# williamyang98/ViterbiDecoderCpp

Hardware: AMD Instinct MI355X
Metric: decoded Mbit/s (= ACS trellis steps/s), update()+chainback(), bit-exact vs scalar reference (higher is better)
Workload: dtype u16

## Files before the change

viterbidecodercpp_amd/csrc/kernels_reg.hpp:

```cpp
#pragma once
#include <hip/hip_runtime.h>
#include <stdint.h>

#include <type_traits>
#include <utility>

#include "common.hpp"

namespace vit {

typedef uint32_t u32;
typedef unsigned short u16x2_t __attribute__((ext_vector_type(2)));
typedef short s16x2_t __attribute__((ext_vector_type(2)));

#define VIT_DEV __device__ __forceinline__

VIT_DEV u32 pk_add(u32 a, u32 b) {
    return __builtin_bit_cast(u32, (u16x2_t)(__builtin_bit_cast(u16x2_t, a) + __builtin_bit_cast(u16x2_t, b)));
}
VIT_DEV u32 pk_sub(u32 a, u32 b) {
    return __builtin_bit_cast(u32, (u16x2_t)(__builtin_bit_cast(u16x2_t, a) - __builtin_bit_cast(u16x2_t, b)));
}
VIT_DEV u32 pk_max_s(u32 a, u32 b) {
    return __builtin_bit_cast(u32, __builtin_elementwise_max(__builtin_bit_cast(s16x2_t, a), __builtin_bit_cast(s16x2_t, b)));
// ... 869 lines not shown
                        constexpr int KV = SP::tail_kind(v % PER);
                        u32 fin;
                        if constexpr (KV == 1) fin = __builtin_amdgcn_perm(pend_acc, pend_f1, SELX32);
                        else if constexpr (KV == 2) fin = __builtin_amdgcn_perm(pend_acc, pend_f1, SELX16);
                        else if constexpr (KV == 3) fin = pend_f1;
                        else if constexpr (KV == 4) fin = __builtin_amdgcn_perm(pend_f1, pend_f2, SELX16);
                        else fin = __builtin_amdgcn_perm(pend_f1, pend_f2, SELX32);
                        dq[v % SPS] = fin;
                        if constexpr (v % SPS == SPS - 1)
                            ws_blk[(v / SPS) * 64 + lane] = make_uint4(dq[0], dq[1], dq[2], dq[3]);
                    };
                    constexpr int KU = SP::tail_kind(UP);
                    constexpr bool DEFER = !GUARDED;
                    if constexpr (DEFER && u > 0) {
                        if constexpr (SP::tail_kind((u - 1) % PER) != 0) finish_tail(std::integral_constant<int, u - 1>{});
                    }
                    if constexpr (KU == 0) {
                        dq[u % SPS] = acc[0];
                        if constexpr (u % SPS == SPS - 1)
                            ws_blk[(u / SPS) * 64 + lane] = make_uint4(dq[0], dq[1], dq[2], dq[3]);
                    } else {
                        pend_acc = acc[0];
                        if constexpr (KU == 1) pend_f1 = (u32)__builtin_amdgcn_ds_bpermute((int)XADDR32, (int)acc[0]);
                        else if constexpr (KU == 2) pend_f1 = (u32)__builtin_amdgcn_ds_bpermute((int)XADDR16, (int)acc[0]);
                        else pend_f1 = (u32)__builtin_amdgcn_ds_bpermute((int)LSWADDR, (int)acc[0]);
                        if constexpr (KU == 4) pend_f2 = (u32)__builtin_amdgcn_ds_bpermute((int)(LSWADDR ^ 128u), (int)acc[0]);
                        if constexpr (KU == 5) pend_f2 = (u32)__builtin_amdgcn_ds_bpermute((int)(LSWADDR ^ 64u), (int)acc[0]);
                        if constexpr (!DEFER) finish_tail(uc);
                    }
                }
                {
                    bool any;
                    if constexpr (EARLY_TEST) {
                        any = early_any != 0;
                    } else if constexpr (NREG >= 64) {
                        const u32 maskq0 = lane < 16 ? BIAS2 : 0u;
                        any = __builtin_amdgcn_ballot_w64(((pk_sub_sat_s_uniform(THRM1B2, m[0]) | FORCE) & maskq0) != 0) != 0;
                    } else {
                        any = __builtin_amdgcn_ballot_w64(pk_max_s(m[0], TLANE) != TCMP) != 0;
                    }
                    if constexpr (NREG >= 64) {
                    if (__builtin_expect(any, 0)) {
                        const u32 maskq = (SP::LANE_BITS == 0 || lane < 16) ? BIAS2 : 0u;
                        const u32 need2 = (pk_sub_sat_s_uniform(THRM1B2, m[0]) | FORCE) & maskq;
                        const u32 nq = SP::LANE_BITS ? (u32)__shfl((int)need2, (int)g) : need2;
                        const u32 msk = ((nq & 0x8000u) ? 0x0000FFFFu : 0u) | ((nq & 0x80000000u) ? 0xFFFF0000u : 0u);
                        u32 mn = m[0];
                        static_for<NREG - 1>([&](auto rc) __attribute__((always_inline)) {
                            mn = pk_min_s(mn, m[decltype(rc)::value + 1]);
                        });
                        if constexpr (SP::LANE_BITS) {
                            mn = pk_min_s(mn, (u32)__shfl_xor((int)mn, 16));
                            mn = pk_min_s(mn, (u32)__shfl_xor((int)mn, 32));
                        }
                        const u32 sub = (mn ^ BIAS2) & msk;
                        static_for<NREG>([&](auto rc) __attribute__((always_inline)) {
                            constexpr int r = decltype(rc)::value;
                            m[r] = pk_sub(m[r], sub);
                        });
                        rsA += (uint64_t)((sub & 0xFFFFu) >> SHIFT);
                        rsB += (uint64_t)((sub >> 16) >> SHIFT);
                    }
                    } else
                    if (__builtin_expect(any, 0)) {
                        u32 mn = m[0];
                        static_for<NREG - 1>([&](auto rc) __attribute__((always_inline)) {
                            mn = pk_min_s(mn, m[decltype(rc)::value + 1]);
                        });
                        u32 sub;
                        if constexpr (SP::LANE_BITS) {
                            const int16_t thr = (int16_t)(uint16_t)(THRM1B2 & 0xFFFFu);
                            uint64_t tA = __builtin_amdgcn_ballot_w64((int16_t)(uint16_t)(m[0] & 0xFFFFu) > thr);
                            uint64_t tB = __builtin_amdgcn_ballot_w64((int16_t)(uint16_t)(m[0] >> 16) > thr);
                            if (a.cfg.threshold == 0) tA = tB = 0xFFFFull;
                            tA &= 0xFFFFull; tB &= 0xFFFFull;
                            tA |= tA << 16; tA |= tA << 32;
                            tB |= tB << 16; tB |= tB << 32;
                            auto s16 = __builtin_amdgcn_permlane16_swap(mn, mn, false, false);
                            mn = pk_min_s(s16[0], s16[1]);
                            auto s32 = __builtin_amdgcn_permlane32_swap(mn, mn, false, false);
                            mn = pk_min_s(s32[0], s32[1]);
                            const u32 unb = mn ^ BIAS2;
                            u32 sa, sb;
                            asm("v_cndmask_b32_e64 %0, 0, %1, %2" : "=v"(sa) : "v"(unb), "s"(tA));
                            asm("v_cndmask_b32_e64 %0, 0, %1, %2" : "=v"(sb) : "v"(unb), "s"(tB));
                            sub = (sa & 0x0000FFFFu) | (sb & 0xFFFF0000u);
                        } else {
                            const u32 need2 = pk_sub_sat_s_uniform(THRM1B2, m[0]) | FORCE;
                            const u32 msk = ((need2 & 0x8000u) ? 0x0000FFFFu : 0u) | ((need2 & 0x80000000u) ? 0xFFFF0000u : 0u);
                            sub = (mn ^ BIAS2) & msk;
                        }
#ifndef VIT_REG_FOLD
#define VIT_REG_FOLD 1
#endif
                        constexpr bool FOLD = VIT_REG_FOLD && SP::LANE_BITS != 0 && !BMCHUNK && !SPLIT && 2 * NPF < NREG;
                        bool folded = false;
                        if constexpr (FOLD) {
                            if ((!GUARDED && u + 1 < U) || t0 + (u32)u + 1u < a.t_end) {
                                static_for<NPF>([&](auto pc) __attribute__((always_inline)) {
                                    constexpr int pp = decltype(pc)::value;
                                    E[(u + 1) & 1][pp] = pk_sub(E[(u + 1) & 1][pp], sub);
                                    EB[(u + 1) & 1][pp] = pk_sub(EB[(u + 1) & 1][pp], sub);
                                });
                                folded = true;
                            }
                        }
                        if (!folded) {
                            static_for<NREG>([&](auto rc) __attribute__((always_inline)) {
                                constexpr int r = decltype(rc)::value;
                                m[r] = pk_sub(m[r], sub);
                            });
                        }
                        rsA += (uint64_t)((sub & 0xFFFFu) >> SHIFT);
                        rsB += (uint64_t)((sub >> 16) >> SHIFT);
                    }
                }
                } else if constexpr (BMCHUNK) {
                    if constexpr (u % GROUP == GROUP - 1) {
                        constexpr int Jb = u / GROUP;
                        constexpr int sl = (Jb + 1) % NG;
                        bm_produce(std::integral_constant<int, GROUP * (Jb + 1)>{}, std::integral_constant<int, sl>{});
                        load_group(t0 + (u32)(GROUP * (Jb + 1 + NG)), std::integral_constant<int, sl>{});
                    }
                    if constexpr (GENERIC) {
                        gen_chunk_row(std::integral_constant<int, u + 1>{}, std::integral_constant<int, 0>{});
                        gen_chunk_row(std::integral_constant<int, u + 1>{}, std::integral_constant<int, 1>{});
                    }
                    static_for<AHEAD>([&](auto ac) __attribute__((always_inline)) { bm_fetch_chunk(std::integral_constant<int, u + 1>{}, ac); });
                }
            }
        });
    };
    if constexpr (RESUME) {
        for (; t0 < a.t_end; t0 += U, ws_blk += (U / SPS) * 64) {
            if (t0 >= T_BEGIN && t0 + U <= a.t_end) block(std::false_type{});
            else block(std::true_type{});
        }
    } else {
        __builtin_amdgcn_s_waitcnt(0x0F70);
        for (; t0 + U <= a.t_end; t0 += U, ws_blk += (U / SPS) * 64) block(std::false_type{});
        if (t0 < a.t_end) block(std::true_type{});
    }

    if constexpr (DW != 4) {
        if (a.t_end % SPS != 0) ws_tile[(size_t)(a.t_end / SPS) * 64 + lane] = make_uint4(dq[0], dq[1], dq[2], dq[3]);
    }

    if (a.metrics_out) {
        const int ph = (int)(a.t_end % SB);
        const int lu = (int)((a.t_end + (u32)PER - 1u) % (u32)PER);
        constexpr size_t N = (size_t)1 << SB;
        static_for<NREG>([&](auto rc) __attribute__((always_inline)) {
            constexpr u32 r = decltype(rc)::value;
            const u32 x = X3 ? SP::slot3(lu, q, r) : ((q << REG_BITS) | r);
            const u32 s = ((x << ph) | (x >> (SB - ph))) & SP::SMASK;
            const u32 v = m[r] ^ BIAS2;
            if (SHIFT) {
                if (validA) ((uint8_t*)a.metrics_out)[(size_t)fA * N + s] = (uint8_t)((v & 0xFFFFu) >> 8);
                if (validB) ((uint8_t*)a.metrics_out)[(size_t)fB * N + s] = (uint8_t)(v >> 24);
            } else {
                if (validA) ((uint16_t*)a.metrics_out)[(size_t)fA * N + s] = (uint16_t)(v & 0xFFFFu);
                if (validB) ((uint16_t*)a.metrics_out)[(size_t)fB * N + s] = (uint16_t)(v >> 16);
            }
        });
    }
    if (a.renorm_sum && q == 0) {
        if (validA) a.renorm_sum[fA] = rsA;
        if (validB) a.renorm_sum[fB] = rsB;
    }
}

struct RegChainbackArgs {
    const uint4* ws;
    size_t ws_tile_stride;
    uint8_t* out;
    const u32* end_state;
    u32 frames, L;
    u32 wave_priority;
};

template <class SP>
VIT_DEV void reg_chainback_coop_body(const RegChainbackArgs& a) {
    static_assert(SP::LANE_BITS == 2 && SP::DW * SP::SPS == 4 && SP::NREG >= 32, "K = 8, 9 layout");
    constexpr int SB = SP::SB, NREG = SP::NREG, REG_BITS = SP::REG_BITS, DW = SP::DW, SPS = SP::SPS;
    constexpr int IGN = SB < 8 ? SB : 8;
    constexpr int SHIFT_STATE = 8 - IGN, SHIFT_TAIL = SB - IGN, TOTAL_BITS = SB + SHIFT_STATE;
    constexpr int PASS = 16;
    constexpr int NBUF = PASS / SPS;
    constexpr int K0 = (((7 - SB) % 8) + 8) % 8;

    const int lane = threadIdx.x & 63;
    const u32 g = lane & 15, q = lane >> 4;
    const size_t tile = blockIdx.x;
    const u32 fA_raw = (u32)tile * 32 + g, fB_raw = fA_raw + 16;
    const bool validA = fA_raw < a.frames, validB = fB_raw < a.frames;
    const u32 fA = validA ? fA_raw : a.frames - 1, fB = validB ? fB_raw : a.frames - 1;
    const uint4* rows = a.ws + tile * a.ws_tile_stride + lane;
    const size_t out_stride = ((size_t)a.L + 7) / 8;
    uint8_t* outA = a.out + (size_t)fA * out_stride;
    uint8_t* outB = a.out + (size_t)fB * out_stride;

    u32 regA = (a.end_state ? (a.end_state[fA] & SP::SMASK) : 0u) << SHIFT_STATE;
    u32 regB = (a.end_state ? (a.end_state[fB] & SP::SMASK) : 0u) << SHIFT_STATE;

    auto trace = [&](u32& reg, const uint4& v, u32 half, u32 ph1, u32 sub) __attribute__((always_inline)) {
        const u32 state = reg >> SHIFT_STATE;
        const u32 x = ((state >> ph1) | (state << (SB - ph1))) & SP::SMASK;
        const u32 qs = x >> REG_BITS, rs = x & (NREG - 1);
        const u32 pos = 32u * (u32)DW * sub + rs + (rs & ~7u) + 8u * half;
        const uint64_t lo64 = ((uint64_t)v.y << 32) | v.x, hi64 = ((uint64_t)v.w << 32) | v.z;
        const uint64_t w64 = (pos & 64u) ? hi64 : lo64;
        const u32 mine = (u32)(w64 >> (pos & 63u)) & 1u;
        const u32 bit = (u32)__shfl((int)mine, (int)(qs * 16 + g));
        reg = (reg >> 1) | (bit << (TOTAL_BITS - 1));
    };
    auto emit = [&](u32 jb) __attribute__((always_inline)) {
        if (q == 0) {
            outA[jb] = (uint8_t)((regA >> SHIFT_TAIL) & 0xFFu);
            outB[jb] = (uint8_t)((regB >> SHIFT_TAIL) & 0xFFu);
        }
    };
    auto slow_step = [&](int t) __attribute__((always_inline)) {
        const uint4 v = rows[(size_t)(t / SPS) * 64];
        const u32 ph1 = (u32)((t + 1) % SB);
        trace(regA, v, 0u, ph1, (u32)(t % SPS));
        trace(regB, v, 1u, ph1, (u32)(t % SPS));
        const int j = t - SB;
        if ((j & 7) == 0) emit((u32)j >> 3);
    };

    int t = (int)a.L - 1 + SB;
    while (t >= SB && (t & 7) != 7) slow_step(t--);
    if (t >= SB && t - (PASS - 1) >= SB) {
        uint4 buf[NBUF];
#pragma unroll
        for (int b = 0; b < NBUF; ++b) buf[b] = rows[(size_t)(t / SPS - b) * 64];
        constexpr int BPP = PASS / 8;
        constexpr int KI = 128 / BPP;
        __shared__ u32 obufA[32 * 64], obufB[32 * 64];
        typedef u32 u32_unaligned __attribute__((aligned(1)));
        u32 ph_run = (u32)((t + 1) % SB);
        while (t - (PASS - 1) >= SB) {
            __builtin_amdgcn_s_waitcnt(0x0F70);
            int it = 0;
            for (; it < KI && t - (PASS - 1) >= SB; ++it, t -= PASS) {
#pragma unroll
                for (int b = 0; b < NBUF; ++b) {
#pragma unroll
                    for (int sidx = SPS - 1; sidx >= 0; --sidx) {
                        const int k = b * SPS + (SPS - 1 - sidx);
                        const u32 ph1 = SB == 8 ? (u32)((8 - (k % 8)) % 8) : ph_run;
                        trace(regA, buf[b], 0u, ph1, (u32)sidx);
                        trace(regB, buf[b], 1u, ph1, (u32)sidx);
                        if (SB != 8) ph_run = ph_run == 0 ? SB - 1 : ph_run - 1;
                        if (k % 8 == K0) {
                            const int slot = 127 - (it * BPP + k / 8);
                            ((uint8_t*)obufA)[(slot >> 2) * 256 + lane * 4 + (slot & 3)] = (uint8_t)((regA >> SHIFT_TAIL) & 0xFFu);
                            ((uint8_t*)obufB)[(slot >> 2) * 256 + lane * 4 + (slot & 3)] = (uint8_t)((regB >> SHIFT_TAIL) & 0xFFu);
                        }
                    }
                    asm volatile("" : "+v"(regA), "+v"(regB) : : "memory");
                    const int nxt = t / SPS - b - NBUF;
                    buf[b] = rows[(size_t)(nxt < 0 ? 0 : nxt) * 64];
                    __builtin_amdgcn_sched_barrier(0);
                }
            }
            if (q == 0) {
                const int nbytes = it * BPP;
                const u32 jb_lo = (u32)(t + PASS - (K0 + 8) - SB) >> 3;
                int sl = 128 - nbytes;
                for (; (sl & 3) != 0 && sl < 128; ++sl) {
                    outA[jb_lo + (u32)(sl - (128 - nbytes))] = ((const uint8_t*)obufA)[(sl >> 2) * 256 + lane * 4 + (sl & 3)];
                    outB[jb_lo + (u32)(sl - (128 - nbytes))] = ((const uint8_t*)obufB)[(sl >> 2) * 256 + lane * 4 + (sl & 3)];
                }
                for (; sl < 128; sl += 4) {
                    *(u32_unaligned*)(outA + jb_lo + (u32)(sl - (128 - nbytes))) = obufA[(sl >> 2) * 64 + lane];
                    *(u32_unaligned*)(outB + jb_lo + (u32)(sl - (128 - nbytes))) = obufB[(sl >> 2) * 64 + lane];
                }
            }
        }
    }
    while (t >= SB) slow_step(t--);
}

#ifndef VIT_REG_CB_RING_DEPTH_K7
#define VIT_REG_CB_RING_DEPTH_K7 4
#endif
constexpr int reg_cb_ring_depth(int nreg, int R) { return nreg == 16 ? (R >= 4 ? 2 : VIT_REG_CB_RING_DEPTH_K7) : 8; }
constexpr int reg_cb_ring_flush_iters(int nreg, int R) { return (nreg == 16 && R >= 4) ? 8 : 16; }
#ifndef VIT_REG_CB_STAGGER
#define VIT_REG_CB_STAGGER 0
#endif
constexpr unsigned reg_cb_ring_slot_bytes() { return 4096u + 4u * (unsigned)VIT_REG_CB_STAGGER; }
constexpr unsigned reg_cb_ring_lds_bytes(int nreg, int R) {
    return (unsigned)reg_cb_ring_depth(nreg, R) * reg_cb_ring_slot_bytes() + (unsigned)reg_cb_ring_flush_iters(nreg, R) * 512u;
}
template <class SP>
VIT_DEV void reg_chainback_ring_body(const RegChainbackArgs& a) {
    static_assert(SP::LANE_BITS == 2 && (SP::NREG == 16 || SP::NREG == 64) && SP::DW * SP::SPS == 4 && SP::SB <= 8, "K = 7, 9 layouts");
    constexpr int SB = SP::SB, REG_BITS = SP::REG_BITS, DW = SP::DW, SPS = SP::SPS;
    constexpr int IGN = SB < 8 ? SB : 8;
    constexpr int SHIFT_STATE = 8 - IGN;
    static_assert(SB - IGN == 0, "... and its low byte is the output byte (shift_tail = 0)");
    constexpr int ITER = 32;
    constexpr int ROWS_IT = ITER / SPS;
    constexpr int D = reg_cb_ring_depth(SP::NREG, SP::R);
    static_assert(ROWS_IT % D == 0, "ring slots are compile-time constants");
    constexpr int KI = reg_cb_ring_flush_iters(SP::NREG, SP::R);
    constexpr int CT = (ITER - 1 + SB) % ITER;
    static_assert(reg_cb_ring_lds_bytes(SP::NREG, SP::R) == D * reg_cb_ring_slot_bytes() + 2 * KI * 64 * 4, "launch size of the ring kernels");
    extern __shared__ uint4 reg_cb_dyn_lds[];
    uint4* const ring = reg_cb_dyn_lds;
    u32* const obuf = (u32*)((char*)reg_cb_dyn_lds + D * reg_cb_ring_slot_bytes());
    typedef __attribute__((address_space(3))) void lds_void_t;
    typedef __attribute__((address_space(1))) const void glb_void_t;
    typedef u32 u32_unaligned __attribute__((aligned(1)));

    const int lane = threadIdx.x & 63;
    const u32 n_tiles = (a.frames + 31u) >> 5;
    const u32 jt = (u32)lane >> 4, g = (u32)lane & 15u;
    const u32 tl_raw = blockIdx.x * 4u + jt;
    const u32 tl = tl_raw < n_tiles ? tl_raw : n_tiles - 1;
    const u32 fA = tl * 32u + g < a.frames ? tl * 32u + g : a.frames - 1;
    const u32 fB = tl * 32u + g + 16u < a.frames ? tl * 32u + g + 16u : a.frames - 1;
    const size_t out_stride = ((size_t)a.L + 7) / 8;
    uint8_t* outA = a.out + (size_t)fA * out_stride;
    uint8_t* outB = a.out + (size_t)fB * out_stride;
    const uint8_t* my_rows = (const uint8_t*)(a.ws + (size_t)tl * a.ws_tile_stride);
    const u32 src_off = (u32)lane * 16u;
    const u32 pair_base = jt * (1024u + (u32)VIT_REG_CB_STAGGER) + g * 16u;

    int t = (int)a.L - 1 + SB;
    const u32 esA = a.end_state ? (a.end_state[fA] & SP::SMASK) : 0u, esB = a.end_state ? (a.end_state[fB] & SP::SMASK) : 0u;
    u32 RA = esA << (24 + SHIFT_STATE), RB = esB << (24 + SHIFT_STATE);
    u32 ph = (u32)(t + 1) % (u32)SB;
    u32 xA = ((esA >> ph) | (esA << (SB - ph))) & SP::SMASK, xB = ((esB >> ph) | (esB << (SB - ph))) & SP::SMASK;
    u32 pos = (SB - ph) % SB;

    auto byte_of = [&](u32 x, u32 base) __attribute__((always_inline)) -> u32 {
        return base + 256u * __builtin_amdgcn_ubfe(x, REG_BITS, 2) + 2u * __builtin_amdgcn_ubfe(x, 3, REG_BITS - 3);
    };
    auto step_back = [&](u32& R, u32& x, u32 byte, u32 p) __attribute__((always_inline)) {
        const u32 bit = __builtin_amdgcn_ubfe(byte, x & 7u, 1);
        R = (R >> 1) | (bit << 31);
        x = (x & ~(1u << p)) | (bit << p);
    };
    auto slow_step = [&](int tt) __attribute__((always_inline)) {
        const uint8_t* row = my_rows + (size_t)(tt / SPS) * 1024u + (u32)(tt % SPS) * (4u * DW);
        const u32 bA = row[byte_of(xA, g * 16u)], bB = row[byte_of(xB, g * 16u) + 1u];
        step_back(RA, xA, bA, pos);
        step_back(RB, xB, bB, pos);
        pos = pos == SB - 1 ? 0u : pos + 1u;
        const int j = tt - SB;
        if ((j & 7) == 0) { outA[j >> 3] = (uint8_t)(RA >> 24); outB[j >> 3] = (uint8_t)(RB >> 24); }
    };

    while (t >= SB && (t & (ITER - 1)) != CT) slow_step(t--);
    if (t - (ITER - 1) >= SB) {
        const uint8_t* tb[4];
#pragma unroll
        for (int jj = 0; jj < 4; ++jj) {
            const u32 tr = blockIdx.x * 4u + (u32)jj;
            tb[jj] = (const uint8_t*)(a.ws + (size_t)(tr < n_tiles ? tr : n_tiles - 1) * a.ws_tile_stride);
        }
        typedef __attribute__((address_space(3))) uint8_t lds_u8_t;
        u32 ring_lds = (u32)(uintptr_t)(lds_u8_t*)ring;
        asm volatile("" : "+s"(ring_lds));
        auto fill = [&](int slot, int row) __attribute__((always_inline)) {
            const u32 vo = src_off + (u32)(row < 0 ? 0 : row) * 1024u;
#pragma unroll
            for (int jj = 0; jj < 4; ++jj)
                __builtin_amdgcn_global_load_lds((glb_void_t*)(tb[jj] + vo), (lds_void_t*)(lds_u8_t*)(uintptr_t)(ring_lds + (u32)slot * reg_cb_ring_slot_bytes() + (u32)jj * (1024u + (u32)VIT_REG_CB_STAGGER)), 16, 0, 0);
        };
        constexpr int S0 = (CT / SPS) % D;
#pragma unroll
        for (int k = 0; k < D; ++k) fill((S0 - k + D) % D, t / SPS - k);
        const uint8_t* ring_b = (const uint8_t*)ring;
        while (t - (ITER - 1) >= SB) {
            __builtin_amdgcn_s_waitcnt(0x0F70);
            const int t0 = t;
            int it = 0;
            for (; it < KI && t - (ITER - 1) >= SB; ++it, t -= ITER) {
#pragma unroll
                for (int pk = 0; pk < ITER; ++pk) {
                    const int cs = CT - pk;
                    const int rk = CT / SPS - (cs >= 0 ? cs / SPS : -((-cs + SPS - 1) / SPS));
                    const int sidx = ((cs % SPS) + SPS) % SPS;
                    const int slot = ((S0 - rk) % D + D) % D;
                    constexpr int NV = 4 * (D - 1);
                    __builtin_amdgcn_s_waitcnt(0x0F70 | (NV & 15) | ((NV >> 4) << 14));
                    const u32 wA = ring_b[slot * (int)reg_cb_ring_slot_bytes() + sidx * 4 * DW + byte_of(xA, pair_base)];
                    const u32 wB = ring_b[slot * (int)reg_cb_ring_slot_bytes() + sidx * 4 * DW + 1 + byte_of(xB, pair_base)];
                    if constexpr (ITER % SB == 0) {
                        const u32 p = (u32)((SB - (((CT - pk + 1) % SB) + SB) % SB) % SB);
                        step_back(RA, xA, wA, p);
                        step_back(RB, xB, wB, p);
                    } else {
                        step_back(RA, xA, wA, pos);
                        step_back(RB, xB, wB, pos);
                        pos = pos == SB - 1 ? 0u : pos + 1u;
                    }
                    if (sidx == 0) {
                        asm volatile("" : "+v"(RA), "+v"(RB), "+v"(xA), "+v"(xB) : : "memory");
                        fill(slot, (t - pk) / SPS - D);
                        __builtin_amdgcn_sched_barrier(0);
                    }
                }
                obuf[it * 64 + lane] = __builtin_amdgcn_perm(RA, RA, 0x00010203u);
                obuf[(KI + it) * 64 + lane] = __builtin_amdgcn_perm(RB, RB, 0x00010203u);
            }
            for (int i = 0; i < it; ++i) {
                const u32 jb = (u32)(t0 - ITER * i - (ITER - 1) - SB) >> 3;
                *(u32_unaligned*)(outA + jb) = obuf[i * 64 + lane];
                *(u32_unaligned*)(outB + jb) = obuf[(KI + i) * 64 + lane];
            }
        }
        __builtin_amdgcn_s_waitcnt(0x0F70);
        if constexpr (ITER % SB == 0) pos = (SB - (u32)(t + 1) % (u32)SB) % SB;
    }
    while (t >= SB) slow_step(t--);
}

template <class SP>
VIT_DEV void reg_chainback16_body(const RegChainbackArgs& a) {
    static_assert(SP::NREG == 16 && SP::DW == 1 && SP::SPS == 4 && SP::SB == 6, "K = 7 layout");
    constexpr int SB = SP::SB;
    constexpr int IGN = SB < 8 ? SB : 8;
    constexpr int SHIFT_STATE = 8 - IGN;
    static_assert(SB - IGN == 0, "shift_tail = 0: the output byte is the 8-bit register itself");
    constexpr int NBUF = 8;

    const int lane = threadIdx.x & 63;
    const u32 n_tiles = (a.frames + 31u) >> 5;
    const u32 p_raw = blockIdx.x * 64 + lane;
    const u32 tile = (p_raw >> 4) < n_tiles ? (p_raw >> 4) : n_tiles - 1, g = p_raw & 15u;
    const u32 fA = tile * 32u + g < a.frames ? tile * 32u + g : a.frames - 1;
    const u32 fB = tile * 32u + g + 16u < a.frames ? tile * 32u + g + 16u : a.frames - 1;
    const uint4* rows = a.ws + (size_t)tile * a.ws_tile_stride + g;
    const size_t out_stride = ((size_t)a.L + 7) / 8;
    uint8_t* outA = a.out + (size_t)fA * out_stride;
    uint8_t* outB = a.out + (size_t)fB * out_stride;
    constexpr u32 SELA = 0x06040200u, SELB = 0x07050301u;

    const u32 esA = a.end_state ? (a.end_state[fA] & SP::SMASK) : 0u, esB = a.end_state ? (a.end_state[fB] & SP::SMASK) : 0u;
    u32 regA = esA << (24 + SHIFT_STATE), regB = esB << (24 + SHIFT_STATE);
    const u32 ph_top = ((u32)a.L + (u32)SB) % (u32)SB;
    u32 xA = ((esA >> ph_top) | (esA << (SB - ph_top))) & SP::SMASK, xB = ((esB >> ph_top) | (esB << (SB - ph_top))) & SP::SMASK;

    auto chase1 = [&](u32& reg, u32& x, u32 lo, u32 hi, u32 p) __attribute__((always_inline)) {
        const u32 w = x > 31u ? hi : lo;
        const u32 bit = __builtin_amdgcn_ubfe(w, x, 1);
        reg = (reg >> 1) | (bit << 31);
        x = (x & ~(1u << p)) | (bit << p);
    };
    auto chase = [&](u32 d0, u32 d1, u32 d2, u32 d3, u32 p) __attribute__((always_inline)) {
        chase1(regA, xA, __builtin_amdgcn_perm(d1, d0, SELA), __builtin_amdgcn_perm(d3, d2, SELA), p);
        chase1(regB, xB, __builtin_amdgcn_perm(d1, d0, SELB), __builtin_amdgcn_perm(d3, d2, SELB), p);
    };
    auto pos_of = [](int t) __attribute__((always_inline)) -> u32 { return (u32)((SB - (t + 1) % SB) % SB); };
    auto emit = [&](u32 jb) __attribute__((always_inline)) {
        outA[jb] = (uint8_t)(regA >> 24);
        outB[jb] = (uint8_t)(regB >> 24);
    };
    auto slow_step = [&](int t) __attribute__((always_inline)) {
        const u32* r32 = (const u32*)(rows + (size_t)(t >> 2) * 64) + (t & 3);
        chase(r32[0], r32[16 * 4], r32[32 * 4], r32[48 * 4], pos_of(t));
        const int j = t - SB;
        if ((j & 7) == 0) emit((u32)j >> 3);
    };

    int t = (int)a.L - 1 + SB;
    while (t >= SB && (((t & 3) != 3) || (((t >> 2) & 1) != 0))) slow_step(t--);
    const int g_top = t >> 2;
    const int g_min = (SB + 3) / 4;
    if (t >= SB && g_top - (NBUF - 1) >= g_min) {
        uint4 buf[NBUF][4];
#pragma unroll
        for (int b = 0; b < NBUF; ++b)
#pragma unroll
            for (int qq = 0; qq < 4; ++qq) buf[b][qq] = rows[(size_t)(g_top - b) * 64 + qq * 16];
        int gb = g_top;
        u32 pos = (u32)__builtin_amdgcn_readfirstlane((int)pos_of(4 * gb + 3));
        constexpr int KI = 32;
        __shared__ uint2 obuf[KI * 64];
        typedef u32 u32_unaligned __attribute__((aligned(1)));
        while (gb - (NBUF - 1) >= g_min) {
            __builtin_amdgcn_s_waitcnt(0x0F70);
            const int gb0 = gb;
            int it = 0;
            for (; it < KI && gb - (NBUF - 1) >= g_min; ++it, gb -= NBUF) {
                u32 accA = 0, accB = 0;
#pragma unroll
                for (int b = 0; b < NBUF; ++b) {
                    const int grp = gb - b;
#pragma unroll
                    for (int sidx = 3; sidx >= 0; --sidx) {
                        const u32 d0 = sidx == 0 ? buf[b][0].x : sidx == 1 ? buf[b][0].y : sidx == 2 ? buf[b][0].z : buf[b][0].w;
                        const u32 d1 = sidx == 0 ? buf[b][1].x : sidx == 1 ? buf[b][1].y : sidx == 2 ? buf[b][1].z : buf[b][1].w;
                        const u32 d2 = sidx == 0 ? buf[b][2].x : sidx == 1 ? buf[b][2].y : sidx == 2 ? buf[b][2].z : buf[b][2].w;
                        const u32 d3 = sidx == 0 ? buf[b][3].x : sidx == 1 ? buf[b][3].y : sidx == 2 ? buf[b][3].z : buf[b][3].w;
                        chase(d0, d1, d2, d3, pos);
                        pos = pos + 1 == (u32)SB ? 0u : pos + 1;
                        if ((b & 1) == 1 && sidx == 2) {
                            accA = (accA << 8) | (regA >> 24);
                            accB = (accB << 8) | (regB >> 24);
                        }
                    }
                    asm volatile("" : "+v"(regA), "+v"(regB), "+v"(xA), "+v"(xB) : : "memory");
                    const int nxt = grp - NBUF;
#pragma unroll
                    for (int qq = 0; qq < 4; ++qq) { typedef u32 u32x4_t __attribute__((ext_vector_type(4))); const u32x4_t v4 = __builtin_nontemporal_load((const u32x4_t*)&rows[(size_t)(nxt < 0 ? 0 : nxt) * 64 + qq * 16]); buf[b][qq] = make_uint4(v4.x, v4.y, v4.z, v4.w); }
                    __builtin_amdgcn_sched_barrier(0);
                }
                obuf[it * 64 + lane] = make_uint2(accA, accB);
            }
            for (int i = 0; i < it; ++i) {
                const uint2 v = obuf[i * 64 + lane];
                const u32 jb = (u32)((gb0 - NBUF * i) / 2 - 4);
                *(u32_unaligned*)(outA + jb) = v.x;
                *(u32_unaligned*)(outB + jb) = v.y;
            }
        }
        t = 4 * gb + 3;
    }
    while (t >= SB) slow_step(t--);
}

template <class SP>
VIT_DEV void reg_chainback0_body(const RegChainbackArgs& a) {
    static_assert(SP::LANE_BITS == 0 && SP::NREG <= 32 && (SP::DW == 1 || SP::DW == 2), "small-K layout");
    constexpr int SB = SP::SB, DW = SP::DW, SPS = SP::SPS;
    constexpr int IGN = SB < 8 ? SB : 8;
    constexpr int SHIFT_STATE = 8 - IGN, SHIFT_TAIL = SB - IGN, TOTAL_BITS = SB + SHIFT_STATE;
    constexpr int NBUF = 32 / SPS;

    const int lane = threadIdx.x & 63;
    const u32 f_raw = blockIdx.x * 64 + lane;
    const bool valid = f_raw < a.frames;
    const u32 f = valid ? f_raw : a.frames - 1;
    const u32 tile = f / SP::TILE, g = f % SP::PAIRS, half = (f % SP::TILE) / SP::PAIRS;
    const uint4* rows = a.ws + (size_t)tile * a.ws_tile_stride + g;
    const size_t out_stride = ((size_t)a.L + 7) / 8;
    uint8_t* out = a.out + (size_t)f * out_stride;
    const u32 hshift = 8u * half;

    u32 reg = (a.end_state ? (a.end_state[f] & SP::SMASK) : 0u) << SHIFT_STATE;
    auto chase = [&](u32 w0, u32 w1, u32 ph1) __attribute__((always_inline)) {
        const u32 state = reg >> SHIFT_STATE;
        const u32 x = ((state >> ph1) | (state << (SB - ph1))) & SP::SMASK;
        const u32 w = (DW == 2 && (x & 16u)) ? w1 : w0;
        const u32 bit = (w >> ((x & 7u) + hshift + 16u * ((x >> 3) & 1u))) & 1u;
        reg = (reg >> 1) | (bit << (TOTAL_BITS - 1));
    };
    auto slow_step = [&](int t) __attribute__((always_inline)) {
        const u32* r32 = (const u32*)(rows + (size_t)(t / SPS) * 64) + (t % SPS) * DW;
        chase(r32[0], DW == 2 ? r32[DW - 1] : 0u, (u32)((t + 1) % SB));
        const int j = t - SB;
        if ((j & 7) == 0) out[(u32)j >> 3] = (uint8_t)((reg >> SHIFT_TAIL) & 0xFFu);
    };

    int t = (int)a.L - 1 + SB;
    while (t >= SB && (t & 7) != 3) slow_step(t--);
    const int g_top = t / SPS;
    const int g_min = (SB + SPS - 1) / SPS;
    if (t >= SB && g_top - (NBUF - 1) >= g_min) {
        uint4 buf[NBUF];
#pragma unroll
        for (int b = 0; b < NBUF; ++b) buf[b] = rows[(size_t)(g_top - b) * 64];
        int gb = g_top;
        u32 ph = (u32)((SPS * gb + SPS - 1 + 1) % SB);
        constexpr int KI = 32;
        __shared__ u32 obuf[KI * 64];
        typedef u32 u32_unaligned __attribute__((aligned(1)));
        constexpr int K_LAST = 24 + (((3 - SB) % 8) + 8) % 8;
        while (gb - (NBUF - 1) >= g_min) {
            __builtin_amdgcn_s_waitcnt(0x0F70);
            const int gb0 = gb;
            int it = 0;
            for (; it < KI && gb - (NBUF - 1) >= g_min; ++it, gb -= NBUF) {
                u32 acc = 0;
#pragma unroll
                for (int b = 0; b < NBUF; ++b) {
#pragma unroll
                    for (int sidx = SPS - 1; sidx >= 0; --sidx) {
                        const int k = b * SPS + (SPS - 1 - sidx);
                        const int c0 = sidx * DW, c1 = sidx * DW + DW - 1;
                        const u32 w0 = c0 == 0 ? buf[b].x : c0 == 1 ? buf[b].y : c0 == 2 ? buf[b].z : buf[b].w;
                        const u32 w1 = c1 == 0 ? buf[b].x : c1 == 1 ? buf[b].y : c1 == 2 ? buf[b].z : buf[b].w;
                        chase(w0, w1, ph);
                        ph = ph == 0 ? SB - 1 : ph - 1;
                        if ((((3 - k - SB) % 8) + 8) % 8 == 0) acc = (acc << 8) | ((reg >> SHIFT_TAIL) & 0xFFu);
                    }
                    asm volatile("" : "+v"(reg) : : "memory");
                    const int nxt = gb - b - NBUF;
                    buf[b] = rows[(size_t)(nxt < 0 ? 0 : nxt) * 64];
                    __builtin_amdgcn_sched_barrier(0);
                }
                obuf[it * 64 + lane] = acc;
            }
            for (int i = 0; i < it; ++i) {
                const int t_top = SPS * (gb0 - NBUF * i) + SPS - 1;
                const u32 jb = (u32)(t_top - K_LAST - SB) >> 3;
                *(u32_unaligned*)(out + jb) = obuf[i * 64 + lane];
            }
        }
        t = SPS * gb + SPS - 1;
    }
    while (t >= SB) slow_step(t--);
}

struct RegExportArgs {
    const u32* ws32;
    size_t ws_tile_stride;
    uint64_t* out;
    u32 frames, n_steps;
};

template <class SP>
VIT_DEV void reg_export_body(const RegExportArgs& a) {
    constexpr int SB = SP::SB, NREG = SP::NREG, REG_BITS = SP::REG_BITS, DW = SP::DW, SPS = SP::SPS;
    constexpr int W = SB >= 6 ? 1 << (SB - 6) : 1;
    const size_t idx = (size_t)blockIdx.x * blockDim.x + threadIdx.x;
    const size_t total = (size_t)a.frames * a.n_steps * W;
    if (idx >= total) return;
    const u32 w = (u32)(idx % W);
    const u32 t = (u32)((idx / W) % a.n_steps);
    const u32 f = (u32)(idx / ((size_t)W * a.n_steps));
    const u32 tile = f / SP::TILE, g = f % SP::PAIRS, half = (f % SP::TILE) / SP::PAIRS;
    const int ph1 = (int)((t + 1) % SB);
    uint64_t word = 0;
    for (u32 b = 0; b < 64; ++b) {
        const u32 s = w * 64 + b;
        if (s > SP::SMASK) break;
        const u32 x = ((s >> ph1) | (s << (SB - ph1))) & SP::SMASK;
        const u32 qs = x >> REG_BITS, rs = x & (NREG - 1);
        const size_t row = (size_t)tile * a.ws_tile_stride + (size_t)(t / SPS) * 64 + qs * SP::PAIRS + g;
        const u32 dwi = (DW == 4) ? (rs >> 4) : (t % SPS) * DW + (rs >> 4);
        const u32 v = a.ws32[row * 4 + dwi];
        word |= (uint64_t)((v >> SP::dec_bit(rs, half)) & 1u) << b;
    }
    a.out[idx] = word;
}

template <class SP>
constexpr int reg_update_min_waves() { return 2; }
#define VIT_REG_UPDATE_IS_CAPPED(K, R) ((K) == 9 || ((K) == 7 && (R) == 3))
#if defined(VIT_REG_TU_K) && VIT_REG_UPDATE_IS_CAPPED(VIT_REG_TU_K, VIT_REG_TU_R)
#define VIT_REG_UPDATE_VGPR_CAP __attribute__((amdgpu_num_vgpr(120)))
#else
#define VIT_REG_UPDATE_VGPR_CAP
#endif
template <class SP, int SHIFT>
__global__ void __launch_bounds__(64, reg_update_min_waves<SP>()) VIT_REG_UPDATE_VGPR_CAP reg_update_kernel(RegUpdateArgs a) {
#ifdef VIT_REG_TU_K
    static_assert(SP::K == VIT_REG_TU_K && SP::R == VIT_REG_TU_R, "the register cap above was chosen for another code");
#endif
#ifdef VIT_HIP_CLOCK_STAMPS
    const uint64_t c0 = __builtin_amdgcn_s_memtime(), r0 = __builtin_amdgcn_s_memrealtime();
#endif
    reg_update_body<SP, SHIFT, false>(a);
#ifdef VIT_HIP_CLOCK_STAMPS
    if (a.stamps && (threadIdx.x & 63) == 0) {
        uint64_t* st = a.stamps + (size_t)blockIdx.x * 6;
        st[0] = c0; st[1] = r0; st[2] = __builtin_amdgcn_s_memtime(); st[3] = __builtin_amdgcn_s_memrealtime();
        st[4] = (uint64_t)__builtin_amdgcn_s_getreg((3 << 11) | 20);
        st[5] = (uint64_t)__builtin_amdgcn_s_getreg((31 << 11) | 4);
    }
#endif
}
template <class SP, int SHIFT>
__global__ void __launch_bounds__(64, 1) reg_resume_kernel(RegUpdateArgs a) { reg_update_body<SP, SHIFT, true>(a); }

template <class SP>
VIT_DEV void reg_chainback_body(const RegChainbackArgs& a) {
    if constexpr (SP::LANE_BITS == 0) reg_chainback0_body<SP>(a);
    else if constexpr (SP::NREG == 16) reg_chainback16_body<SP>(a);
    else if constexpr (SP::NREG == 64) reg_chainback_ring_body<SP>(a);
    else reg_chainback_coop_body<SP>(a);
}
constexpr unsigned reg_chainback_dyn_lds_bytes(int K, int R, bool alt) {
    return (K == 9 && !alt) ? reg_cb_ring_lds_bytes(64, R) : (K == 7 && alt) ? reg_cb_ring_lds_bytes(16, R) : 0u;
}
constexpr unsigned reg_chainback_frames_per_block(int K) { return (K == 7 || K == 9) ? 128u : K < 7 ? 64u : 32u; }
template <class SP>
constexpr int reg_chainback_min_waves() { return SP::NREG == 64 ? 1 : 2; }
template <class SP>
__global__ void __launch_bounds__(64, reg_chainback_min_waves<SP>()) reg_chainback_kernel(RegChainbackArgs a) {
    if (a.wave_priority) __builtin_amdgcn_s_setprio(3);
    reg_chainback_body<SP>(a);
}
template <class SP>
VIT_DEV void reg_chainback_alt_body(const RegChainbackArgs& a) {
    if constexpr (SP::NREG == 64) reg_chainback_coop_body<SP>(a);
    else if constexpr (SP::NREG == 16 && SP::LANE_BITS == 2) reg_chainback_ring_body<SP>(a);
}
template <class SP>
constexpr int reg_chainback_alt_min_waves() { return SP::NREG == 16 ? 1 : 2; }
template <class SP>
__global__ void __launch_bounds__(64, reg_chainback_alt_min_waves<SP>()) reg_chainback_alt_kernel(RegChainbackArgs a) { reg_chainback_alt_body<SP>(a); }
template <class SP>
__global__ void reg_export_kernel(RegExportArgs a) { reg_export_body<SP>(a); }

}
```

Baseline: 157,900.

## Track chainback state as LDS offset bits and sign-extended masks in ring kernel

The ring chainback now keeps the traceback state split into an LDS byte offset and a 3-bit in-word index, updated in place with bfi/alignbit. This removes the per-step recomputation of the byte address from the state. The iteration length becomes lcm(32, SB) so the bit position inside the shift register is a compile-time constant, and the loop is fully unrolled through static_for. The register chainback also switches from a shift position to a rotating mask and uses sbfe plus alignbit. The tradeoffs are larger unrolled code and a fallback path when the dynamic LDS base is not 1024-aligned.

Result: slower. 143,000 (-9.4%).

```diff
diff --git a/viterbidecodercpp_amd/csrc/kernels_reg.hpp b/viterbidecodercpp_amd/csrc/kernels_reg.hpp
--- a/viterbidecodercpp_amd/csrc/kernels_reg.hpp
+++ b/viterbidecodercpp_amd/csrc/kernels_reg.hpp
@@ -1195,14 +1195,18 @@
     constexpr int IGN = SB < 8 ? SB : 8;
     constexpr int SHIFT_STATE = 8 - IGN;
     static_assert(SB - IGN == 0, "... and its low byte is the output byte (shift_tail = 0)");
-    constexpr int ITER = 32;
+    constexpr int ITER = clcm(32, SB);
+    constexpr int NDW = ITER / 32;
     constexpr int ROWS_IT = ITER / SPS;
     constexpr int D = reg_cb_ring_depth(SP::NREG, SP::R);
     static_assert(ROWS_IT % D == 0, "ring slots are compile-time constants");
-    constexpr int KI = reg_cb_ring_flush_iters(SP::NREG, SP::R);
-    constexpr int CT = (ITER - 1 + SB) % ITER;
-    static_assert(reg_cb_ring_lds_bytes(SP::NREG, SP::R) == D * reg_cb_ring_slot_bytes() + 2 * KI * 64 * 4, "launch size of the ring kernels");
-    extern __shared__ uint4 reg_cb_dyn_lds[];
+    constexpr int KDW = reg_cb_ring_flush_iters(SP::NREG, SP::R);
+    constexpr int KI = KDW / NDW;
+    static_assert(KI >= 1, "the parking area holds one iteration");
+    constexpr int TOPMOD = clcm(8, SB), CT = SB - 1;
+    static_assert(TOPMOD % SPS == 0 && ITER % TOPMOD == 0, "an iteration ends where the next one can start");
+    static_assert(reg_cb_ring_lds_bytes(SP::NREG, SP::R) == D * reg_cb_ring_slot_bytes() + 2 * KDW * 64 * 4, "launch size of the ring kernels");
+    extern __shared__ __attribute__((aligned(1024))) uint4 reg_cb_dyn_lds[];
     uint4* const ring = reg_cb_dyn_lds;
     u32* const obuf = (u32*)((char*)reg_cb_dyn_lds + D * reg_cb_ring_slot_bytes());
     typedef __attribute__((address_space(3))) void lds_void_t;
@@ -1248,68 +1252,86 @@
         if ((j & 7) == 0) { outA[j >> 3] = (uint8_t)(RA >> 24); outB[j >> 3] = (uint8_t)(RB >> 24); }
     };
 
-    while (t >= SB && (t & (ITER - 1)) != CT) slow_step(t--);
-    if (t - (ITER - 1) >= SB) {
+    while (t >= SB && t % TOPMOD != CT) slow_step(t--);
+    typedef __attribute__((address_space(3))) uint8_t lds_u8_t;
+    u32 ring_lds = (u32)(uintptr_t)(lds_u8_t*)ring;
+    asm volatile("" : "+s"(ring_lds));
+    if (t - (ITER - 1) >= SB && (ring_lds & 1023u) == 0) {
         const uint8_t* tb[4];
 #pragma unroll
         for (int jj = 0; jj < 4; ++jj) {
             const u32 tr = blockIdx.x * 4u + (u32)jj;
             tb[jj] = (const uint8_t*)(a.ws + (size_t)(tr < n_tiles ? tr : n_tiles - 1) * a.ws_tile_stride);
         }
-        typedef __attribute__((address_space(3))) uint8_t lds_u8_t;
-        u32 ring_lds = (u32)(uintptr_t)(lds_u8_t*)ring;
-        asm volatile("" : "+s"(ring_lds));
         auto fill = [&](int slot, int row) __attribute__((always_inline)) {
             const u32 vo = src_off + (u32)(row < 0 ? 0 : row) * 1024u;
 #pragma unroll
             for (int jj = 0; jj < 4; ++jj)
                 __builtin_amdgcn_global_load_lds((glb_void_t*)(tb[jj] + vo), (lds_void_t*)(lds_u8_t*)(uintptr_t)(ring_lds + (u32)slot * reg_cb_ring_slot_bytes() + (u32)jj * (1024u + (u32)VIT_REG_CB_STAGGER)), 16, 0, 0);
         };
-        constexpr int S0 = (CT / SPS) % D;
 #pragma unroll
-        for (int k = 0; k < D; ++k) fill((S0 - k + D) % D, t / SPS - k);
-        const uint8_t* ring_b = (const uint8_t*)ring;
+        for (int k = 0; k < D; ++k) fill(k, t / SPS - k);
+        constexpr u32 HI_BITS = (1u << (REG_BITS - 3)) - 1u;
+        static_assert(((3u * (1024u + (u32)VIT_REG_CB_STAGGER) | 0xF0u) & (0x300u | (HI_BITS << 1) | 1u)) == 0, "the chased bits of the offset are clear in the pair's base");
+        auto offset_of = [&](u32 x) __attribute__((always_inline)) -> u32 {
+            return ring_lds + pair_base + 256u * __builtin_amdgcn_ubfe(x, REG_BITS, 2) + 2u * __builtin_amdgcn_ubfe(x, 3, REG_BITS - 3);
+        };
+        u32 oA = offset_of(xA), oB = offset_of(xB) + 1u, iA = xA & 7u, iB = xB & 7u;
+        auto step_back = [&](u32& R, u32& o, u32& i, u32 byte, int pk) __attribute__((always_inline)) {
+            const int p = pk % SB, g0 = pk - p;
+            const bool whole = g0 / 32 == (g0 + 2) / 32;
+            const u32 d = (u32)__builtin_amdgcn_sbfe((int)byte, i, 1);
+            if (p == 0) {
+                asm("v_bfi_b32 %0, 1, %1, %0" : "+v"(i) : "v"(d));
+                if (!whole) R = __builtin_amdgcn_alignbit(d, R, 1);
+            } else if (p < 3) {
+                i = (d & (1u << p)) | (i & ~(1u << p));
+                if (!whole) R = __builtin_amdgcn_alignbit(d, R, 1);
+                else if (p == 2) R = __builtin_amdgcn_alignbit(i, R, 3);
+            } else {
+                const u32 m = 1u << (p < REG_BITS ? p - 2 : p - REG_BITS + 8);
+                o = (d & m) | (o & ~m);
+                R = __builtin_amdgcn_alignbit(d, R, 1);
+            }
+        };
         while (t - (ITER - 1) >= SB) {
             __builtin_amdgcn_s_waitcnt(0x0F70);
             const int t0 = t;
             int it = 0;
             for (; it < KI && t - (ITER - 1) >= SB; ++it, t -= ITER) {
-#pragma unroll
-                for (int pk = 0; pk < ITER; ++pk) {
-                    const int cs = CT - pk;
-                    const int rk = CT / SPS - (cs >= 0 ? cs / SPS : -((-cs + SPS - 1) / SPS));
-                    const int sidx = ((cs % SPS) + SPS) % SPS;
-                    const int slot = ((S0 - rk) % D + D) % D;
+                static_for<ITER>([&](auto pkc) __attribute__((always_inline)) {
+                    constexpr int pk = decltype(pkc)::value;
+                    constexpr int cs = CT - pk;
+                    constexpr int rk = CT / SPS - (cs >= 0 ? cs / SPS : -((-cs + SPS - 1) / SPS));
+                    constexpr int sidx = ((cs % SPS) + SPS) % SPS;
+                    constexpr int slot = rk % D;
                     constexpr int NV = 4 * (D - 1);
                     __builtin_amdgcn_s_waitcnt(0x0F70 | (NV & 15) | ((NV >> 4) << 14));
-                    const u32 wA = ring_b[slot * (int)reg_cb_ring_slot_bytes() + sidx * 4 * DW + byte_of(xA, pair_base)];
-                    const u32 wB = ring_b[slot * (int)reg_cb_ring_slot_bytes() + sidx * 4 * DW + 1 + byte_of(xB, pair_base)];
-                    if constexpr (ITER % SB == 0) {
-                        const u32 p = (u32)((SB - (((CT - pk + 1) % SB) + SB) % SB) % SB);
-                        step_back(RA, xA, wA, p);
-                        step_back(RB, xB, wB, p);
-                    } else {
-                        step_back(RA, xA, wA, pos);
-                        step_back(RB, xB, wB, pos);
-                        pos = pos == SB - 1 ? 0u : pos + 1u;
-                    }
+                    const u32 wA = ((const lds_u8_t*)(uintptr_t)oA)[slot * (int)reg_cb_ring_slot_bytes() + sidx * 4 * DW];
+                    const u32 wB = ((const lds_u8_t*)(uintptr_t)oB)[slot * (int)reg_cb_ring_slot_bytes() + sidx * 4 * DW];
+                    step_back(RA, oA, iA, wA, pk);
+                    step_back(RB, oB, iB, wB, pk);
                     if (sidx == 0) {
-                        asm volatile("" : "+v"(RA), "+v"(RB), "+v"(xA), "+v"(xB) : : "memory");
+                        asm volatile("" : "+v"(RA), "+v"(RB), "+v"(oA), "+v"(oB), "+v"(iA), "+v"(iB) : : "memory");
                         fill(slot, (t - pk) / SPS - D);
                         __builtin_amdgcn_sched_barrier(0);
                     }
-                }
-                obuf[it * 64 + lane] = __builtin_amdgcn_perm(RA, RA, 0x00010203u);
-                obuf[(KI + it) * 64 + lane] = __builtin_amdgcn_perm(RB, RB, 0x00010203u);
+                    if (pk % 32 == 31) {
+                        obuf[(it * NDW + pk / 32) * 64 + lane] = __builtin_amdgcn_perm(RA, RA, 0x00010203u);
+                        obuf[(KDW + it * NDW + pk / 32) * 64 + lane] = __builtin_amdgcn_perm(RB, RB, 0x00010203u);
+                    }
+                });
             }
-            for (int i = 0; i < it; ++i) {
-                const u32 jb = (u32)(t0 - ITER * i - (ITER - 1) - SB) >> 3;
-                *(u32_unaligned*)(outA + jb) = obuf[i * 64 + lane];
-                *(u32_unaligned*)(outB + jb) = obuf[(KI + i) * 64 + lane];
+            for (int n = 0; n < it * NDW; ++n) {
+                const u32 jb = (u32)(t0 - 32 * n - 31 - SB) >> 3;
+                *(u32_unaligned*)(outA + jb) = obuf[n * 64 + lane];
+                *(u32_unaligned*)(outB + jb) = obuf[(KDW + n) * 64 + lane];
             }
         }
         __builtin_amdgcn_s_waitcnt(0x0F70);
-        if constexpr (ITER % SB == 0) pos = (SB - (u32)(t + 1) % (u32)SB) % SB;
+        xA = (__builtin_amdgcn_ubfe(oA, 8, 2) << REG_BITS) | (__builtin_amdgcn_ubfe(oA, 1, REG_BITS - 3) << 3) | iA;
+        xB = (__builtin_amdgcn_ubfe(oB, 8, 2) << REG_BITS) | (__builtin_amdgcn_ubfe(oB, 1, REG_BITS - 3) << 3) | iB;
+        pos = (SB - (u32)(t + 1) % (u32)SB) % SB;
     }
     while (t >= SB) slow_step(t--);
 }
@@ -1340,15 +1362,15 @@
     const u32 ph_top = ((u32)a.L + (u32)SB) % (u32)SB;
     u32 xA = ((esA >> ph_top) | (esA << (SB - ph_top))) & SP::SMASK, xB = ((esB >> ph_top) | (esB << (SB - ph_top))) & SP::SMASK;
 
-    auto chase1 = [&](u32& reg, u32& x, u32 lo, u32 hi, u32 p) __attribute__((always_inline)) {
+    auto chase1 = [&](u32& reg, u32& x, u32 lo, u32 hi, u32 m) __attribute__((always_inline)) {
         const u32 w = x > 31u ? hi : lo;
-        const u32 bit = __builtin_amdgcn_ubfe(w, x, 1);
-        reg = (reg >> 1) | (bit << 31);
-        x = (x & ~(1u << p)) | (bit << p);
-    };
-    auto chase = [&](u32 d0, u32 d1, u32 d2, u32 d3, u32 p) __attribute__((always_inline)) {
-        chase1(regA, xA, __builtin_amdgcn_perm(d1, d0, SELA), __builtin_amdgcn_perm(d3, d2, SELA), p);
-        chase1(regB, xB, __builtin_amdgcn_perm(d1, d0, SELB), __builtin_amdgcn_perm(d3, d2, SELB), p);
+        const u32 d = (u32)__builtin_amdgcn_sbfe((int)w, x, 1);
+        reg = __builtin_amdgcn_alignbit(d, reg, 1);
+        x = (d & m) | (x & ~m);
+    };
+    auto chase = [&](u32 d0, u32 d1, u32 d2, u32 d3, u32 m) __attribute__((always_inline)) {
+        chase1(regA, xA, __builtin_amdgcn_perm(d1, d0, SELA), __builtin_amdgcn_perm(d3, d2, SELA), m);
+        chase1(regB, xB, __builtin_amdgcn_perm(d1, d0, SELB), __builtin_amdgcn_perm(d3, d2, SELB), m);
     };
     auto pos_of = [](int t) __attribute__((always_inline)) -> u32 { return (u32)((SB - (t + 1) % SB) % SB); };
     auto emit = [&](u32 jb) __attribute__((always_inline)) {
@@ -1357,7 +1379,7 @@
     };
     auto slow_step = [&](int t) __attribute__((always_inline)) {
         const u32* r32 = (const u32*)(rows + (size_t)(t >> 2) * 64) + (t & 3);
-        chase(r32[0], r32[16 * 4], r32[32 * 4], r32[48 * 4], pos_of(t));
+        chase(r32[0], r32[16 * 4], r32[32 * 4], r32[48 * 4], 1u << pos_of(t));
         const int j = t - SB;
         if ((j & 7) == 0) emit((u32)j >> 3);
     };
@@ -1373,7 +1395,7 @@
 #pragma unroll
             for (int qq = 0; qq < 4; ++qq) buf[b][qq] = rows[(size_t)(g_top - b) * 64 + qq * 16];
         int gb = g_top;
-        u32 pos = (u32)__builtin_amdgcn_readfirstlane((int)pos_of(4 * gb + 3));
+        u32 msk = (u32)__builtin_amdgcn_readfirstlane((int)(1u << pos_of(4 * gb + 3)));
         constexpr int KI = 32;
         __shared__ uint2 obuf[KI * 64];
         typedef u32 u32_unaligned __attribute__((aligned(1)));
@@ -1392,8 +1414,8 @@
                         const u32 d1 = sidx == 0 ? buf[b][1].x : sidx == 1 ? buf[b][1].y : sidx == 2 ? buf[b][1].z : buf[b][1].w;
                         const u32 d2 = sidx == 0 ? buf[b][2].x : sidx == 1 ? buf[b][2].y : sidx == 2 ? buf[b][2].z : buf[b][2].w;
                         const u32 d3 = sidx == 0 ? buf[b][3].x : sidx == 1 ? buf[b][3].y : sidx == 2 ? buf[b][3].z : buf[b][3].w;
-                        chase(d0, d1, d2, d3, pos);
-                        pos = pos + 1 == (u32)SB ? 0u : pos + 1;
+                        chase(d0, d1, d2, d3, msk);
+                        msk = msk == 1u << (SB - 1) ? 1u : msk << 1;
                         if ((b & 1) == 1 && sidx == 2) {
                             accA = (accA << 8) | (regA >> 24);
                             accB = (accB << 8) | (regB >> 24);
```
